# RhushabhVaghela/Custom-NVComp-with-ZSTD

Hardware: AMD Instinct MI355X
Metric: compress GB/s + ratio, 1 GB @ level 3, 64 KB chunks; libzstd round-trip OK (higher is better)
Workload: dtype u8; 1 GPU; C3: 16384 x 64 KiB chunks (1.00 GiB), level 3, independent frames; chunk_bytes=65536, chunks_total=16384, chunks_rank0=16384, level=3, parallelism=dp1 (contiguous chunk shards, RCCL all-gather of sizes inside the step), gathered_frame_bytes=388747049

## Files before the change

### custom-nvcomp-with-zstd_amd/csrc/zh_common.h

```cpp
#pragma once
#include <hip/hip_runtime.h>
#include <stdint.h>
#include "zstd_hip_params.h"
#include "zh_dict_ent.h"
#include "zh_block_plan.h"

typedef int16_t s16;
typedef int32_t s32;

#define ZH_STATS_LIT 0u
#define ZH_STATS_LL 256u
#define ZH_STATS_OF 320u
#define ZH_STATS_ML 384u
#define ZH_STATS_WORDS 448u

#define ZH_SEQ_CAP 13120u
#define ZH_SEQ_BYTES (ZH_SEQ_CAP * 8u)
#define ZH_K3_W 1u
#define ZH_K3_SEGS (21u * ZH_K3_W)
#define ZH_K3_SLOTS (64u * ZH_K3_W)
#define ZH_K3_RUN 16u
#define ZH_K3_SLOT(t, g) (3u * (g) + (t))
#define ZH_K3_TSTRIDE ZH_K3_RUN
#define ZH_K3_SEGLEN(nbseq) ((((nbseq) + ZH_K3_SEGS - 1u) / ZH_K3_SEGS + ZH_K3_RUN - 1u) & ~(ZH_K3_RUN - 1u))
// ... 29 lines not shown
  u8 *base;
  u32 *ctr;
  const u16 *dtab;
  u32 dtab_P;
  const u32 *dd_prev;
  const u32 *dd_head;
  u32 dd_pre, dd_split;
  u8 *deep_slots;
  u32 deep_nslots;
  const ZhDictEnt *dent;
  u32 *stats;
  __device__ u64 *seq(u32 b) const { return (u64 *)(base + (size_t)b * ZH_WS_BLOCK_BYTES); }
  __device__ u8 *lits(u32 b) const { return base + (size_t)b * ZH_WS_BLOCK_BYTES + ZH_SEQ_BYTES; }
  __device__ u32 *meta(u32 b) const { return (u32 *)(base + (size_t)b * ZH_WS_BLOCK_BYTES + ZH_SEQ_BYTES + ZH_LIT_BYTES); }
  __device__ u32 *dbg(u32 b) const { return meta(b) + 4; }
  __device__ u8 *fse(u32 b) const { return base + (size_t)b * ZH_WS_BLOCK_BYTES + ZH_SEQ_BYTES + ZH_LIT_BYTES + ZH_META_BYTES; }
  __device__ u32 *fsef(u32 b) const { return (u32 *)(fse(b) + ZH_FSE_FIELDS); }
};

#define ZH_DTAB_MARGIN 256u

struct ZhClassRanges {
  u32 range[ZH_NCLASSES][2];
  u32 ctr[4];
};
#define ZH_RANGE_CTR_DEEP 3u

__host__ __device__ __forceinline__ u32 zh_k3_magic(u32 L) { return ((1u << 24) + L - 1u) / L; }
__device__ __forceinline__ u32 zh_k3_index(u32 e, u32 t, u32 L, u32 m) {
  u32 const g = __umulhi(e << 8, m), r = e - g * L;
// ... 26 lines not shown
```

### custom-nvcomp-with-zstd_amd/csrc/zh_entropy.hip

```cpp
#include "zh_common.h"

namespace {

constexpr u32 K2_THREADS = 128;
constexpr u32 SW_WORDS = 184;

constexpr u32 OFF_SW = 0;
constexpr u32 OFF_HVAL = OFF_SW + 4 * SW_WORDS;
constexpr u32 OFF_HNB = OFF_HVAL + 2 * 256;
constexpr u32 OFF_MISC = OFF_HNB + 256;
constexpr u32 OFF_HIST = OFF_MISC + 4 * 64;
constexpr u32 OFF_HBUF = OFF_HIST + 4 * 256;
constexpr u32 OFF_SCR = OFF_HBUF + 768;
constexpr u32 OFF_U = OFF_SCR + 1024;
static_assert(OFF_U % 16 == 0, "alignment");
constexpr u32 OFF_NODES = OFF_U;
constexpr u32 U_HUF_END = OFF_NODES + 8 * 516;
constexpr u32 OFF_ST_LL = OFF_U;
constexpr u32 OFF_ST_OF = OFF_ST_LL + 1024;
constexpr u32 OFF_ST_ML = OFF_ST_OF + 512;
constexpr u32 OFF_SYM = OFF_ST_ML + 1024;
constexpr u32 SYM_OF = 36, SYM_ML = 68;
constexpr u32 OFF_TSYM = OFF_SYM + 976;
constexpr u32 OFF_NORM = OFF_TSYM + 512;
// ... 848 lines not shown
    sz[k] = (wave_sum(bits) + 1 + 7) >> 3;
    cs += sz[k];
  }
  u32 const fl = 1 + (nl > 31) + (nl > 4095);
  u32 const other = (cLit == 0 || cLit >= nl - minGain) ? fl + nl : cLit == 1 ? fl + 1 : lhSize + cLit;
  if (lhSize + cs > other) return false;
  wave_sync();
  ((u32 *)hnb)[lane] = ((const u32 *)dent->hnb)[lane];
  ((u32 *)hval)[lane] = ((const u32 *)dent->hval)[lane];
  ((u32 *)hval)[64 + lane] = ((const u32 *)dent->hval)[64 + lane];
  if (lane == 0) { ssz[0] = sz[0]; ssz[1] = sz[1]; ssz[2] = sz[2]; ssz[3] = sz[3]; ssz[4] = cs; }
  wave_sync();
  return true;
}

extern "C" __global__ __launch_bounds__(K2_THREADS) void zh_entropy_kernel(const ZhBlockDesc *__restrict__ blocks, ZhWorkspace ws, u32 window_log,
                                                                             u32 cfg_block_size, u64 *__restrict__ item_size,
                                                                             u32 *__restrict__ item_status, u32 *__restrict__ blk_size,
                                                                             const u8 *__restrict__ blk_level) {
  extern __shared__ __attribute__((aligned(16))) u8 smem_all[];
  u32 const wave = threadIdx.x >> 6;
  u8 *const smem = smem_all + wave * K2_W1;
  u32 *const xch = (u32 *)(smem_all + OFF_MISC) + 56;
  u32 *sw = (u32 *)(smem + OFF_SW);
  u32 *misc = (u32 *)(smem + OFF_MISC);
  u32 *hist = (u32 *)(smem + OFF_HIST);
  u16 *hval = (u16 *)(smem + OFF_HVAL);
  u8 *hnb = smem + OFF_HNB;
  u8 *hbuf = smem + OFF_HBUF;
  HufNode *nodes = (HufNode *)(smem + OFF_NODES);
  u16 *stLL = (u16 *)(smem + OFF_ST_LL), *stOF = (u16 *)(smem + OFF_ST_OF), *stML = (u16 *)(smem + OFF_ST_ML);
  FseSym *symLL = (FseSym *)(smem + OFF_SYM), *symOF = symLL + SYM_OF, *symML = symLL + SYM_ML;
  u8 *tsym = smem + OFF_TSYM;
  s16 *norm = (s16 *)(smem + OFF_NORM);
  u8 *wts = smem + OFF_WTS;
  SerialScratch *scr = (SerialScratch *)(smem + OFF_SCR);

  u32 const b = blockIdx.x, lane = lane_id();
  ZhBlockDesc const d = blocks[b];
  u32 const n = d.n;
  if (n == 0) return;
  const u32 *meta = ws.meta(b);
  u32 const nseq_raw = meta[0], nlit = meta[1], rle = meta[2] == 1u, k1hist = meta[2] == ZH_META_K1HIST;
  Out const o{d.dst, d.dst_cap};
  constexpr u32 DENT_FLAGS = ZH_F_FIRST | ZH_F_DICT | ZH_F_DICTENT;
  const ZhDictEnt *const dent = (d.flags & DENT_FLAGS) == DENT_FLAGS ? ws.dent : nullptr;
  u32 *const stats = (d.flags & ZH_F_STATS) ? ws.stats : nullptr;
  u32 const lit_min = stats ? 1u : (dent && !k1hist) ? ZH_DENT_LITERALS_MIN : ZH_COMPRESS_LITERALS_SIZE_MIN + 1u;
  if (wave == 0 && lane == 0) sw[0] = 0;
#ifdef ZH_STAMPS
  u64 stamp_prev = __builtin_amdgcn_s_memtime();
  u32 st[12] = {0, 0, 0, 0, 0, 0, 0, 0, 0, 0, 0, 0};
#endif
// ... 514 lines not shown
        total = finish_block(d, o, blk, op, false);
      }
    }
  }
  ZH_STAMP(8);
#ifdef ZH_STAMPS
  if (lane == 0) {
    u32 *dbg = ws.dbg(b);
    if (wave == 0) { for (int k = 0; k < 4; k++) dbg[6 + k] = st[k]; dbg[42] = st[11]; }
    else { for (int k = 4; k < 9; k++) dbg[6 + k] = st[k]; dbg[17] = st[9]; dbg[18] = st[10]; dbg[19] = nseq_raw; }
  }
#endif
  if (wave == 1 && !handoff) write_status(d, b, total, item_size, item_status, blk_size);
}

constexpr u32 K3_SEGS = ZH_K3_SEGS;
constexpr u32 K3_W = ZH_K3_W;
constexpr u32 K3_OCC = 8;
constexpr u32 K3_WARM = 128;
constexpr u32 K3_WAVES = K3_W == 1 ? 4 : K3_W;
constexpr u32 K3_BPW = K3_WAVES / K3_W;
constexpr u32 K3_TAB_STRIDE = (ZH_FSE_TAB_BYTES + 15) & ~15u;
constexpr u32 K3_LDS = K3_BPW * K3_TAB_STRIDE + 64;
constexpr u32 K3_BATCH = 16;
constexpr u32 K3_TABW = ZH_FSE_TAB_BYTES / 4;

__device__ __forceinline__ void k3_chain(ZhWorkspace ws, u32 bb, u8 *smem, u32 lane, u32 *xw) {
#ifdef ZH_STAMPS
  u64 const k3pre = __builtin_amdgcn_s_memtime();
  u64 const k3rt0 = __builtin_amdgcn_s_memrealtime();
// ... 118 lines not shown
    k3rerun += __builtin_popcountll(__ballot(active));
#endif
    if (active) {
      entry = ne;
      u32 s = ne;
      if (!pass(s, true)) x = s;
    }
  }
  if (g == K3_SEGS - 1 && lane < 3 * K3_SEGS) ff[ZH_FF_SLL + t] = x;
#ifdef ZH_STAMPS
  if (lane == 0) { u32 *dbg = ws.dbg(bb); dbg[46] = (u32)(__builtin_amdgcn_s_memtime() - k3t0); dbg[47] = k3rounds; dbg[48] = k3rerun; dbg[49] = nbSeq;
                   dbg[50] = (u32)(k3t0 - k3pre); dbg[51] = (u32)k3rt0; dbg[52] = (u32)__builtin_amdgcn_s_memrealtime(); }
#endif
}

extern "C" __global__ __launch_bounds__(64 * K3_WAVES) __attribute__((amdgpu_waves_per_eu(K3_OCC, 8))) void zh_fse_chain_kernel(const ZhBlockDesc *__restrict__ blocks, u32 nblocks, ZhWorkspace ws) {
  extern __shared__ __attribute__((aligned(16))) u8 smem_all[];
  u32 const bw = threadIdx.x / (64 * K3_W), lane = threadIdx.x % (64 * K3_W);
  u32 const bb = blockIdx.x * K3_BPW + bw;
  if (bb >= nblocks || blocks[bb].n == 0) return;
  if (ws.fsef(bb)[ZH_FF_NEED] == 0) return;
  k3_chain(ws, bb, smem_all + bw * K3_TAB_STRIDE, lane, (u32 *)(smem_all + K3_BPW * K3_TAB_STRIDE));
}

constexpr u32 KP_SW = 0, KP_DNB = 4 * SW_WORDS, KP_LDS = (KP_DNB + 4 * 128 + 15) & ~15u;
constexpr u32 K4_WAVES = 4;
constexpr u32 K4_PF = 1;

__device__ __forceinline__ void k4_pack(const ZhBlockDesc &d, ZhWorkspace ws, u32 b, u8 *smem, u32 lane, u64 *__restrict__ item_size,
                                        u32 *__restrict__ item_status, u32 *__restrict__ blk_size) {
  const u32 *ff = ws.fsef(b);
  u32 *sw = (u32 *)(smem + KP_SW);
  u32 *dNb = (u32 *)(smem + KP_DNB);
  const u8 *fz = ws.fse(b);
  if (lane < 36) dNb[lane] = ((const FseSym *)(fz + ZH_FT_SYLL))[lane].dNb;
  if (lane < 32) dNb[40 + lane] = ((const FseSym *)(fz + ZH_FT_SYOF))[lane].dNb;
  if (lane < 53) dNb[72 + lane] = ((const FseSym *)(fz + ZH_FT_SYML))[lane].dNb;
// ... 40 lines not shown
    }
    u32 v6[6] = {vOF, vML, vLL, ll, mlb, ob};
    u32 n6[6] = {nOF, nML, nLL, valid ? llbits : 0u, valid ? mlbits : 0u, ofc};
    sink_append<6>(bs, o, sw, v6, n6);
  }
  {
    u32 v3[3] = {sML, sOF, sLL};
    u32 n3[3] = {lane == 0 ? logML : 0u, lane == 0 ? logOF : 0u, lane == 0 ? logLL : 0u};
    sink_append<3>(bs, o, sw, v3, n3);
  }
  sink_close(bs, o, sw);
  u32 const total = finish_block(d, o, blk, bs.pos, false);
  write_status(d, b, total, item_size, item_status, blk_size);
}

extern "C" __global__ __launch_bounds__(64 * K4_WAVES) void zh_seq_pack_kernel(const ZhBlockDesc *__restrict__ blocks, u32 nblocks, ZhWorkspace ws,
                                                                               u64 *__restrict__ item_size, u32 *__restrict__ item_status,
                                                                               u32 *__restrict__ blk_size) {
  extern __shared__ __attribute__((aligned(16))) u8 smem_all[];
  u32 const wv = threadIdx.x >> 6, b = blockIdx.x * K4_WAVES + wv;
  if (b >= nblocks) return;
  ZhBlockDesc const d = blocks[b];
  if (d.n == 0 || ws.fsef(b)[ZH_FF_NEED] == 0) return;
  k4_pack(d, ws, b, smem_all + wv * KP_LDS, lane_id(), item_size, item_status, blk_size);
}

extern "C" u32 zh_entropy_lds_bytes() { return K2_LDS; }
#ifdef ZH_STAMPS
extern "C" __global__ void zh_read_hst(u32 *out) { for (int k = 0; k < 6; k++) { out[k] = g_hst[k]; g_hst[k] = 0; } }
extern "C" void zh_hst_host(u32 *out6) {
  u32 *d = nullptr;
  if (hipMalloc(&d, 24) != hipSuccess) return;
  hipLaunchKernelGGL(zh_read_hst, dim3(1), dim3(1), 0, 0, d);
  (void)hipMemcpy(out6, d, 24, hipMemcpyDeviceToHost);
  (void)hipFree(d);
}
#endif

namespace zh {
hipError_t entropy_init() {
  hipError_t e = hipFuncSetAttribute((const void *)zh_entropy_kernel, hipFuncAttributeMaxDynamicSharedMemorySize, (int)K2_LDS);
  if (e == hipSuccess) e = hipFuncSetAttribute((const void *)zh_fse_chain_kernel, hipFuncAttributeMaxDynamicSharedMemorySize, (int)K3_LDS);
  return e;
}
void entropy_launch(const ZhBlockDesc *d_descs, u32 nblocks, ZhWorkspace ws, u32 window_log, u32 cfg_block_size, u64 *d_item_size,
                    u32 *d_item_status, u32 *d_blk_size, const u8 *d_blk_level, hipStream_t stream) {
  hipLaunchKernelGGL(zh_entropy_kernel, dim3(nblocks), dim3(K2_THREADS), K2_LDS, stream, d_descs, ws, window_log, cfg_block_size, d_item_size,
                     d_item_status, d_blk_size, d_blk_level);
  u32 const g3 = (nblocks + K3_BPW - 1) / K3_BPW, g4 = (nblocks + K4_WAVES - 1) / K4_WAVES;
  hipLaunchKernelGGL(zh_fse_chain_kernel, dim3(g3), dim3(64 * K3_WAVES), K3_LDS, stream, d_descs, nblocks, ws);
  hipLaunchKernelGGL(zh_seq_pack_kernel, dim3(g4), dim3(64 * K4_WAVES), K4_WAVES * KP_LDS, stream, d_descs, nblocks, ws, d_item_size,
                     d_item_status, d_blk_size);
}
}
```

### custom-nvcomp-with-zstd_amd/csrc/zh_host.cpp

```cpp
#include <hip/hip_runtime.h>
#include <dlfcn.h>
#if defined(__SANITIZE_ADDRESS__)
#define ZH_DLOPEN_DEEPBIND 0
#elif defined(__has_feature)
#if __has_feature(address_sanitizer)
#define ZH_DLOPEN_DEEPBIND 0
#endif
#endif
#ifndef ZH_DLOPEN_DEEPBIND
#define ZH_DLOPEN_DEEPBIND RTLD_DEEPBIND
#endif

#include <algorithm>
#include <chrono>
#include <cstring>
#include <mutex>
#include <new>
#include <vector>

#include "cuda_zstd_adaptive.h"
#include "cuda_zstd_hybrid.h"
#include "cuda_zstd_manager.h"
#include "cuda_zstd_nvcomp.h"
#include "zh_adaptive.h"
// ... 284 lines not shown
struct WsLayout {
  size_t descs, items, blk_size, item_size, item_status, staging, counter, blocks, deep, deep_slots, total;
  size_t ldm_table, ldm_skey, ldm_sslot, ldm_scount, ldm_rec;
  size_t rank, blk_level, ranges;
  BatchShape shape;
  explicit WsLayout(const BatchShape &s) : shape(s) {
    size_t const nblocks = s.nblocks, nitems = s.nitems, cells = s.ldm_cells;
    size_t o = 0;
    auto take = [&o](size_t bytes) { size_t const at = o; o = align256(o + bytes); return at; };
    descs = take(nblocks * sizeof(ZhBlockDesc));
    items = take(nitems * sizeof(ZhItemDesc));
    blk_size = take(nblocks * 4);
    item_size = take(nitems * 8);
    item_status = take(nitems * 4);
    staging = take(s.staged ? nblocks * (size_t)ZH_STAGE_SLOT : 0);
    counter = take(4);
    blocks = take(nblocks * (size_t)ZH_WS_BLOCK_BYTES);
    deep_slots = s.deep ? std::min(nblocks, (size_t)ZH_DEEP_SLOTS_MAX) : 0;
    deep = take(deep_slots * ZH_DEEP_SLOT_BYTES);
    ldm_table = take(cells ? sizeof(u64) << s.ldm_tlog : 0);
    ldm_skey = take(cells * ZH_LDM_CELL_SAMPLES * sizeof(u64));
    ldm_sslot = take(cells * ZH_LDM_CELL_SAMPLES * sizeof(u32));
    ldm_scount = take(cells * sizeof(u32));
    ldm_rec = take(cells * sizeof(ZhLdmRecord));
    rank = take(s.levels ? nitems * 4 : 0);
    blk_level = take(s.levels ? nblocks : 0);
    ranges = take(s.levels ? sizeof(ZhClassRanges) : 0);
    total = o + 256;
  }
};

// ... 168 lines not shown
    a.dict = d;
    a.dict_n = n;
    a.dict_off = (u32)off;
    a.dict_id = id;
  }
};

ZhBatch bind_batch(const WsLayout &L, u8 *base, const DevDict *dd, const CompressionConfig &c, u32 *stats = nullptr) {
  if (dd && !dd->n) dd = nullptr;
  ZhBatch b{};
  b.descs = (ZhBlockDesc *)(base + L.descs);
  b.items = (ZhItemDesc *)(base + L.items);
  b.item_size = (u64 *)(base + L.item_size);
  b.item_status = (u32 *)(base + L.item_status);
  b.blk_size = (u32 *)(base + L.blk_size);
  b.nblocks = (u32)L.shape.nblocks;
  b.nitems = (u32)L.shape.nitems;
  b.block_size = c.block_size;
  b.level = c.level;
  b.gather = L.shape.staged;
  b.checksum = c.checksum != ChecksumPolicy::NO_COMPUTE_NO_VERIFY;
  b.window_log = L.shape.levels ? 0u : c.window_log;
  const ZhDictEnt *const dent = dd ? dd->dent(c) : nullptr;
  b.plan.flags = (b.checksum ? ZH_F_CHECKSUM : 0u) | (dent ? ZH_F_DICTENT : 0u) | (stats ? ZH_F_STATS : 0u);
  b.plan.hist = L.shape.levels || c.window_log >= ZH_HIST_WINDOW_LOG;
  if (dd) {
    b.plan.dict = dd->content();
    b.plan.dict_n = (u32)dd->content_n();
    b.plan.dict_id = dd->id;
  }
// ... 1998 lines not shown
}
long long cuda_zstd_hip_ldm_plan(cuda_zstd_manager_t *m, const void *d_src, size_t size, unsigned int *host_records, size_t capacity,
                                 void *workspace, size_t workspace_size, hipStream_t stream) {
  if (!m || !m->manager) return -1;
  size_t n = 0;
  Status const s = m->manager->ldm_plan(d_src, size, host_records, capacity, &n, workspace, workspace_size, stream);
  if (s != Status::SUCCESS) { (void)c_err(s); return -1; }
  return (long long)n;
}
void cuda_zstd_hip_ldm_profile(int on, double *ms) {
  double const t = zh::ldm_profile(on != 0);
  if (ms) *ms = t;
}
void cuda_zstd_hip_profile_enable(int on) { zh::profile_enable(on != 0); }
int cuda_zstd_hip_profile_collect(double *ms3) { return zh::profile_collect(ms3); }

struct cuda_zstd_stream_t {
  std::unique_ptr<ZstdStreamingManager> m;
};
cuda_zstd_stream_t *cuda_zstd_stream_create(int level) {
  if (!is_valid_compression_level(level)) return nullptr;
  try {
    auto *h = new cuda_zstd_stream_t;
    h->m.reset(new ZstdStreamingManager(CompressionConfig::from_level(level)));
    return h;
  } catch (...) {
    return nullptr;
  }
}
void cuda_zstd_stream_destroy(cuda_zstd_stream_t *s) { delete s; }
// ... 179 lines not shown
```

### custom-nvcomp-with-zstd_amd/csrc/zh_launch.h

```cpp
#pragma once
#include "zh_common.h"
#include "zh_ldm.h"

struct ZhDecArgs {
  const void *const *in_ptrs;
  const void *one_in;
  u64 one_in_size;
  void *one_out;
  const size_t *in_sizes;
  void *const *out_ptrs;
  const size_t *out_caps;
  u64 out_cap_all;
  size_t *out_sizes;
  u32 *statuses;
  u8 *ws;
  u64 slot_bytes;
  u32 lit_bytes, block_cap, seq_cap, nvcomp_codes;
  u32 ho_off;
  const u8 *dict;
  u64 dict_n;
  u32 dict_off;
  u32 dict_id;
};
#define ZH_DEC_HANDOFF_BYTES 5376u

struct ZhBatch {
  ZhBlockDesc *descs;
  ZhItemDesc *items;
  u64 *item_size;
  u32 *item_status;
  u32 *blk_size;
  ZhBatchPlan plan;
  ZhWorkspace ws;
  u32 *rank;
  u8 *blk_level;
  ZhClassRanges *ranges;
  u32 nblocks, nitems;
  u32 window_log, block_size;
  int level;
  bool gather, checksum;
};

struct ZhPlanArrays {
  const void *const *in_ptrs;
  const size_t *in_sizes;
  void *const *out_ptrs;
  const int *levels;
};

namespace zh {
u32 dec_lds_bytes();
hipError_t launch_decompress(const ZhDecArgs &a, u32 nitems, hipStream_t stream);
hipError_t launch_decompress_sizes(const ZhDecArgs &a, u32 nitems, hipStream_t stream);
hipError_t init_kernels();
u32 lz_lds_bytes();
u32 entropy_lds_bytes();
hipError_t lz_dict_tables(const u8 *content, size_t cn, u16 *out, u32 *tmp32, u32 &P, hipStream_t stream);
hipError_t lz_deep_dict_tables(const u8 *content, size_t cn, u8 *stg, u32 *dprev, u32 *dhead, u32 &P, u32 &split, hipStream_t stream);
hipError_t launch_compress(const ZhBatch &b, hipStream_t stream);
void profile_enable(bool on);
int profile_collect(double *totals);
#define ZH_RANK_MAX_ITEMS (1u << 20)
hipError_t launch_plan(const ZhBatch &b, const ZhPlanArrays &a, hipStream_t stream);
hipError_t ldm_launch(const u8 *src, u64 size, u32 ncells, u32 table_log, u32 max_dist, u32 flags, u64 *table, u64 *skey, u32 *sslot,
                      u32 *scount, ZhBlockDesc *descs, u8 *staging, u32 *blk_size, ZhLdmRecord *rec, hipStream_t stream);
double ldm_profile(bool on);
}
```

### custom-nvcomp-with-zstd_amd/csrc/zh_plan.hip

```cpp
#include "zh_common.h"
#include "zh_launch.h"
#include "zh_scan.h"
#include "zh_xxh64.h"

#include <mutex>
#include <vector>

extern "C" u32 zh_lz_lds_bytes();
extern "C" u32 zh_entropy_lds_bytes();
namespace zh {
hipError_t lz_init();
void lz_launch(const ZhBlockDesc *d_descs, u32 nblocks, ZhWorkspace ws, u32 mode, hipStream_t stream);
void lz_launch_ranged(const ZhBlockDesc *d_descs, u32 nblocks, ZhWorkspace ws, ZhClassRanges *d_ranges, hipStream_t stream);
hipError_t lz_deep_init();
hipError_t lz_deep_launch(const ZhBlockDesc *d_descs, u32 nblocks, ZhWorkspace ws, int level, hipStream_t stream);
hipError_t lz_deep_launch_ranged(const ZhBlockDesc *d_descs, u32 nblocks, ZhWorkspace ws, ZhClassRanges *d_ranges, const u8 *d_blk_level,
                                 hipStream_t stream);
hipError_t entropy_init();
void entropy_launch(const ZhBlockDesc *d_descs, u32 nblocks, ZhWorkspace ws, u32 window_log, u32 cfg_block_size, u64 *d_item_size,
                    u32 *d_item_status, u32 *d_blk_size, const u8 *d_blk_level, hipStream_t stream);
}

__device__ inline void zh_plan_block(const ZhBatch &B, const ZhPlanArrays &a, u32 i, u32 k, u32 b, int level, bool valid) {
  ZhPlanItem const it{(const u8 *)a.in_ptrs[i], a.in_sizes[i], i, level, (u8 *)a.out_ptrs[i]};
  ZhBlockDesc d = zh_block_desc(B.plan, it, k, b);
  if (!valid) d.n = 0;
  B.descs[b] = d;
  if (k != 0) return;
  bool invalid;
  B.items[i] = zh_item_desc(B.plan, it, b, &invalid);
  if (invalid || !valid) { B.item_size[i] = 0; B.item_status[i] = ZH_ST_INVALID; }
}

extern "C" __global__ void zh_plan_kernel(ZhBatch B, ZhPlanArrays a) {
  u32 const t = blockIdx.x * blockDim.x + threadIdx.x, bpi = B.nblocks / B.nitems;
// ... 46 lines not shown
    cr->range[tid][1] = b1 * bpi;
    if (tid <= ZH_CLASS_DEEP0) cr->ctr[tid] = b0 * bpi;
  }
}

extern "C" __global__ void zh_plan_levels_kernel(ZhBatch B, ZhPlanArrays a) {
  u32 const t = blockIdx.x * blockDim.x + threadIdx.x, bpi = B.nblocks / B.nitems;
  if (t >= B.nblocks) return;
  u32 const i = t / bpi, k = t % bpi, b = B.rank[i] * bpi + k;
  int const level = a.levels[i];
  bool const valid = ZH_LEVEL_VALID(level);
  zh_plan_block(B, a, i, k, b, level, valid);
  B.blk_level[b] = valid ? (u8)level : (u8)0;
}
static_assert(ZH_LEVEL_WINDOW_LOG(1) >= ZH_HIST_WINDOW_LOG, "every level's frames may reach the previous block");

extern "C" __global__ __launch_bounds__(256) void zh_gather_kernel(const ZhItemDesc *__restrict__ items, const ZhBlockDesc *__restrict__ descs,
                                                                    const u32 *__restrict__ blk_size, u64 *item_size, u32 *item_status) {
  u32 const b = blockIdx.x, tid = threadIdx.x;
  ZhBlockDesc const d = descs[b];
  if (d.n == 0 && !(d.flags & ZH_F_LDM)) return;
  ZhItemDesc const id = items[d.item];
  if (id.nblocks <= 1) return;
  u32 const k = b - id.first_block;
  __shared__ u64 part[2][4];
  __shared__ u32 badp[4];
  u64 pre = 0, tot = 0;
  u32 bad = 0;
  for (u32 j = tid; j < id.nblocks; j += 256) {
    u32 const s = blk_size[id.first_block + j];
// ... 37 lines not shown
  if (size + 4 > id.cap) {
    if (lane == 0) item_status[it] = ZH_ST_TOO_SMALL;
    return;
  }
  if (lane < 4) id.dst[size + lane] = (u8)(h >> (8 * lane));
  if (lane == 0) item_size[it] = size + 4;
}

namespace zh {

hipError_t init_kernels() {
  hipError_t e = lz_init();
  if (e != hipSuccess) return e;
  e = lz_deep_init();
  if (e != hipSuccess) return e;
  return entropy_init();
}

u32 lz_lds_bytes() { return zh_lz_lds_bytes(); }
u32 entropy_lds_bytes() { return zh_entropy_lds_bytes(); }

namespace {
struct ProfState {
  std::mutex mu;
  bool on = false;
  std::vector<hipEvent_t> pool;
  std::vector<std::vector<hipEvent_t>> pending;
};
ProfState &prof() {
  static ProfState p;
// ... 20 lines not shown
  int n = 0;
  for (auto &ev : p.pending) {
    (void)hipEventSynchronize(ev[3]);
    float a = 0, b = 0, c = 0;
    (void)hipEventElapsedTime(&a, ev[0], ev[1]);
    (void)hipEventElapsedTime(&b, ev[1], ev[2]);
    (void)hipEventElapsedTime(&c, ev[2], ev[3]);
    totals[0] += a; totals[1] += b; totals[2] += c;
    for (auto e : ev) p.pool.push_back(e);
    n++;
  }
  p.pending.clear();
  return n;
}

hipError_t launch_compress(const ZhBatch &b, hipStream_t stream) {
  if (b.nblocks == 0) return hipSuccess;
  std::vector<hipEvent_t> ev;
  {
    std::lock_guard<std::mutex> g(prof().mu);
    if (prof().on) for (int k = 0; k < 4; k++) ev.push_back(prof_event());
  }
  if (!ev.empty()) (void)hipEventRecord(ev[0], stream);
  if (b.ranges) {
    lz_launch_ranged(b.descs, b.nblocks, b.ws, b.ranges, stream);
    hipError_t const e = lz_deep_launch_ranged(b.descs, b.nblocks, b.ws, b.ranges, b.blk_level, stream);
    if (e != hipSuccess) return e;
  } else if (b.level >= ZH_DEEP_LEVEL) {
    (void)hipMemsetAsync(b.ws.ctr, 0, 4, stream);
    hipError_t const e = lz_deep_launch(b.descs, b.nblocks, b.ws, b.level, stream);
    if (e != hipSuccess) return e;
  } else {
    (void)hipMemsetAsync(b.ws.ctr, 0, 4, stream);
    lz_launch(b.descs, b.nblocks, b.ws, (u32)ZH_K1_MODE(b.level), stream);
  }
  if (!ev.empty()) (void)hipEventRecord(ev[1], stream);
  entropy_launch(b.descs, b.nblocks, b.ws, b.window_log, b.block_size, b.item_size, b.item_status, b.blk_size, b.blk_level, stream);
  if (!ev.empty()) (void)hipEventRecord(ev[2], stream);
  if (b.gather && b.nitems)
    hipLaunchKernelGGL(zh_gather_kernel, dim3(b.nblocks), dim3(256), 0, stream, b.items, b.descs, b.blk_size, b.item_size, b.item_status);
  if (b.checksum && b.nitems)
    hipLaunchKernelGGL(zh_checksum_kernel, dim3(b.nitems), dim3(64), 0, stream, b.items, b.descs, b.item_size, b.item_status);
  if (!ev.empty()) {
    (void)hipEventRecord(ev[3], stream);
    std::lock_guard<std::mutex> g(prof().mu);
    prof().pending.push_back(ev);
  }
  return hipGetLastError();
}

hipError_t launch_plan(const ZhBatch &b, const ZhPlanArrays &a, hipStream_t stream) {
  if (!b.nblocks) return hipSuccess;
// ... 13 lines not shown
```

### custom-nvcomp-with-zstd_amd/cuda_zstd/__init__.py

```python
from __future__ import annotations

import ctypes
import os
from typing import List, Sequence

_HERE = os.path.dirname(os.path.abspath(__file__))
LIB_PATH = os.environ.get("CUDA_ZSTD_HIP_LIB") or os.path.join(os.path.dirname(_HERE), "libcuda_zstd_hip.so")

OK, INVALID, OOM, DEVICE_ERROR, CORRUPT, TOO_SMALL, CHECKSUM, COMPRESSION = 0, 2, 3, 4, 6, 7, 10, 12

_lib = None


class ZstdError(RuntimeError):
    def __init__(self, code: int, what: str = ""):
        self.code = code
        super().__init__(f"{what}: {error_string(code)} (code {code})")


def lib() -> ctypes.CDLL:
    global _lib
    if _lib is None:
        if not os.path.exists(LIB_PATH):
            raise ImportError(f"{LIB_PATH} not found: build it with __graft_entry__.build() (make -C custom-nvcomp-with-zstd_amd)")
# ... 1005 lines not shown
    rc = lib().cuda_zstd_extract_metadata(ptr, n, ctypes.byref(lv), ctypes.byref(us), ctypes.byref(did), ctypes.byref(ck))
    del keep
    if rc:
        raise ZstdError(rc, "cuda_zstd_extract_metadata")
    return {"level": lv.value, "uncompressed_size": us.value, "dictionary_id": did.value, "checksum": bool(ck.value)}


def profile_enable(on: bool = True) -> None:
    lib().cuda_zstd_hip_profile_enable(1 if on else 0)


def profile_collect():
    ms = (ctypes.c_double * 3)()
    n = lib().cuda_zstd_hip_profile_collect(ms)
    return n, list(ms)
```

### include/cuda_zstd_capi.h

```cpp
#ifndef CUDA_ZSTD_CAPI_H_
#define CUDA_ZSTD_CAPI_H_

#include <hip/hip_runtime_api.h>
#include <stddef.h>

#ifdef __cplusplus
extern "C" {
#endif

typedef struct cuda_zstd_manager_t cuda_zstd_manager_t;
typedef struct cuda_zstd_dict_t cuda_zstd_dict_t;

cuda_zstd_manager_t *cuda_zstd_create_manager(int compression_level);
void cuda_zstd_destroy_manager(cuda_zstd_manager_t *manager);
int cuda_zstd_compress(cuda_zstd_manager_t *manager, const void *src, size_t src_size, void *dst, size_t *dst_size,
                       void *workspace, size_t workspace_size, hipStream_t stream);
int cuda_zstd_decompress(cuda_zstd_manager_t *manager, const void *src, size_t src_size, void *dst, size_t *dst_size,
                         void *workspace, size_t workspace_size, hipStream_t stream);
size_t cuda_zstd_get_compress_workspace_size(cuda_zstd_manager_t *manager, size_t src_size);
size_t cuda_zstd_get_decompress_workspace_size(cuda_zstd_manager_t *manager, size_t compressed_size);
cuda_zstd_dict_t *cuda_zstd_train_dictionary(const void **samples, const size_t *sample_sizes, size_t num_samples, size_t dict_size);
cuda_zstd_dict_t *cuda_zstd_train_dictionary_params(const void **samples, const size_t *sample_sizes, size_t num_samples,
                                                    size_t dict_size, unsigned k, unsigned d);
size_t cuda_zstd_train_dictionary_device_get_temp_size(size_t total_sample_bytes, size_t num_samples, size_t dict_size, unsigned k);
// ... 149 lines not shown
int cuda_zstd_adaptive_select_level(const void *d_data, size_t size, size_t sample_bytes, int preference,
                                    cuda_zstd_adaptive_stats_t *h_out, hipStream_t stream);
int cuda_zstd_adaptive_finalize_host(const unsigned *hist256, unsigned sample_size, unsigned repeated_pairs, unsigned max_run_length,
                                     unsigned pattern_score, int preference, cuda_zstd_adaptive_stats_t *out);

int cuda_zstd_set_long_distance(cuda_zstd_manager_t *manager, int enable, unsigned window_log, unsigned hash_log);
int cuda_zstd_set_dict_entropy(cuda_zstd_manager_t *manager, int enable);
int cuda_zstd_set_checksum(cuda_zstd_manager_t *manager, int enable);
long long cuda_zstd_hip_ldm_plan(cuda_zstd_manager_t *manager, const void *d_src, size_t size, unsigned int *host_records, size_t capacity,
                                 void *workspace, size_t workspace_size, hipStream_t stream);
void cuda_zstd_hip_ldm_profile(int on, double *ms);

const char *cuda_zstd_hip_version(void);
void cuda_zstd_hip_profile_enable(int on);
int cuda_zstd_hip_profile_collect(double *ms3);
void cuda_zstd_hip_dict_train_profile(int on, double *ms3);
unsigned int cuda_zstd_hip_kernel_lds_bytes(int which);

#ifdef __cplusplus
}
#endif
#endif
```

Measured before the change: 91.55 GB/s.

## Schedule entropy kernels over blocks sorted by estimated cost

Adds a key, counting-sort and scatter pass after LZ matching that buckets blocks by a cost estimate from their metadata (sequence and literal counts). The three entropy kernels then dispatch workgroups through this order, so the heaviest blocks start first and the tail imbalance should shrink. The ordering only runs above a block-count threshold and when more than one bucket is occupied. It costs three extra small launches, including a single-workgroup sort, and one extra indirection per block, and it reuses the blk_size buffer as sort scratch.

```diff
diff --git a/custom-nvcomp-with-zstd_amd/csrc/zh_common.h b/custom-nvcomp-with-zstd_amd/csrc/zh_common.h
--- a/custom-nvcomp-with-zstd_amd/csrc/zh_common.h
+++ b/custom-nvcomp-with-zstd_amd/csrc/zh_common.h
@@ -67,6 +67,16 @@
   __device__ u8 *lits(u32 b) const { return base + (size_t)b * ZH_WS_BLOCK_BYTES + ZH_SEQ_BYTES; }
   __device__ u32 *meta(u32 b) const { return (u32 *)(base + (size_t)b * ZH_WS_BLOCK_BYTES + ZH_SEQ_BYTES + ZH_LIT_BYTES); }
   __device__ u32 *dbg(u32 b) const { return meta(b) + 4; }
+  __device__ u32 *order(u32 s) const { return meta(s) + 3; }
+  __device__ bool order_useful() const {
+    u64 const active = ((u64)ctr[2] << 32 | ctr[1]) & ~(1ull << 63);
+    return (active & (active - 1)) != 0;
+  }
+  template <bool ORD>
+  __device__ u32 dispatch(u32 s) const {
+    if constexpr (ORD) return order_useful() ? *order(s) : s;
+    else return s;
+  }
   __device__ u8 *fse(u32 b) const { return base + (size_t)b * ZH_WS_BLOCK_BYTES + ZH_SEQ_BYTES + ZH_LIT_BYTES + ZH_META_BYTES; }
   __device__ u32 *fsef(u32 b) const { return (u32 *)(fse(b) + ZH_FSE_FIELDS); }
 };
diff --git a/custom-nvcomp-with-zstd_amd/csrc/zh_entropy.hip b/custom-nvcomp-with-zstd_amd/csrc/zh_entropy.hip
--- a/custom-nvcomp-with-zstd_amd/csrc/zh_entropy.hip
+++ b/custom-nvcomp-with-zstd_amd/csrc/zh_entropy.hip
@@ -886,10 +886,10 @@
   return true;
 }
 
-extern "C" __global__ __launch_bounds__(K2_THREADS) void zh_entropy_kernel(const ZhBlockDesc *__restrict__ blocks, ZhWorkspace ws, u32 window_log,
-                                                                             u32 cfg_block_size, u64 *__restrict__ item_size,
-                                                                             u32 *__restrict__ item_status, u32 *__restrict__ blk_size,
-                                                                             const u8 *__restrict__ blk_level) {
+template <bool ORD>
+__device__ __forceinline__ void k2_block(const ZhBlockDesc *__restrict__ blocks, ZhWorkspace ws, u32 window_log, u32 cfg_block_size,
+                                         u64 *__restrict__ item_size, u32 *__restrict__ item_status, u32 *__restrict__ blk_size,
+                                         const u8 *__restrict__ blk_level) {
   extern __shared__ __attribute__((aligned(16))) u8 smem_all[];
   u32 const wave = threadIdx.x >> 6;
   u8 *const smem = smem_all + wave * K2_W1;
@@ -908,7 +908,7 @@
   u8 *wts = smem + OFF_WTS;
   SerialScratch *scr = (SerialScratch *)(smem + OFF_SCR);
 
-  u32 const b = blockIdx.x, lane = lane_id();
+  u32 const b = ws.dispatch<ORD>(blockIdx.x), lane = lane_id();
   ZhBlockDesc const d = blocks[b];
   u32 const n = d.n;
   if (n == 0) return;
@@ -1453,6 +1453,19 @@
   if (wave == 1 && !handoff) write_status(d, b, total, item_size, item_status, blk_size);
 }
 
+extern "C" __global__ __launch_bounds__(K2_THREADS) void zh_entropy_kernel(const ZhBlockDesc *__restrict__ blocks, ZhWorkspace ws, u32 window_log,
+                                                                             u32 cfg_block_size, u64 *__restrict__ item_size,
+                                                                             u32 *__restrict__ item_status, u32 *__restrict__ blk_size,
+                                                                             const u8 *__restrict__ blk_level) {
+  k2_block<false>(blocks, ws, window_log, cfg_block_size, item_size, item_status, blk_size, blk_level);
+}
+extern "C" __global__ __launch_bounds__(K2_THREADS) void zh_entropy_ordered_kernel(const ZhBlockDesc *__restrict__ blocks, ZhWorkspace ws,
+                                                                                     u32 window_log, u32 cfg_block_size, u64 *__restrict__ item_size,
+                                                                                     u32 *__restrict__ item_status, u32 *__restrict__ blk_size,
+                                                                                     const u8 *__restrict__ blk_level) {
+  k2_block<true>(blocks, ws, window_log, cfg_block_size, item_size, item_status, blk_size, blk_level);
+}
+
 constexpr u32 K3_SEGS = ZH_K3_SEGS;
 constexpr u32 K3_W = ZH_K3_W;
 constexpr u32 K3_OCC = 8;
@@ -1601,13 +1614,22 @@
 #endif
 }
 
-extern "C" __global__ __launch_bounds__(64 * K3_WAVES) __attribute__((amdgpu_waves_per_eu(K3_OCC, 8))) void zh_fse_chain_kernel(const ZhBlockDesc *__restrict__ blocks, u32 nblocks, ZhWorkspace ws) {
+template <bool ORD>
+__device__ __forceinline__ void k3_workgroup(const ZhBlockDesc *__restrict__ blocks, u32 nblocks, ZhWorkspace ws) {
   extern __shared__ __attribute__((aligned(16))) u8 smem_all[];
   u32 const bw = threadIdx.x / (64 * K3_W), lane = threadIdx.x % (64 * K3_W);
-  u32 const bb = blockIdx.x * K3_BPW + bw;
-  if (bb >= nblocks || blocks[bb].n == 0) return;
+  u32 const slot = blockIdx.x * K3_BPW + bw;
+  if (slot >= nblocks) return;
+  u32 const bb = ws.dispatch<ORD>(slot);
+  if (blocks[bb].n == 0) return;
   if (ws.fsef(bb)[ZH_FF_NEED] == 0) return;
   k3_chain(ws, bb, smem_all + bw * K3_TAB_STRIDE, lane, (u32 *)(smem_all + K3_BPW * K3_TAB_STRIDE));
+}
+extern "C" __global__ __launch_bounds__(64 * K3_WAVES) __attribute__((amdgpu_waves_per_eu(K3_OCC, 8))) void zh_fse_chain_kernel(const ZhBlockDesc *__restrict__ blocks, u32 nblocks, ZhWorkspace ws) {
+  k3_workgroup<false>(blocks, nblocks, ws);
+}
+extern "C" __global__ __launch_bounds__(64 * K3_WAVES) __attribute__((amdgpu_waves_per_eu(K3_OCC, 8))) void zh_fse_chain_ordered_kernel(const ZhBlockDesc *__restrict__ blocks, u32 nblocks, ZhWorkspace ws) {
+  k3_workgroup<true>(blocks, nblocks, ws);
 }
 
 constexpr u32 KP_SW = 0, KP_DNB = 4 * SW_WORDS, KP_LDS = (KP_DNB + 4 * 128 + 15) & ~15u;
@@ -1678,15 +1700,26 @@
   write_status(d, b, total, item_size, item_status, blk_size);
 }
 
+template <bool ORD>
+__device__ __forceinline__ void k4_workgroup(const ZhBlockDesc *__restrict__ blocks, u32 nblocks, ZhWorkspace ws, u64 *__restrict__ item_size,
+                                             u32 *__restrict__ item_status, u32 *__restrict__ blk_size) {
+  extern __shared__ __attribute__((aligned(16))) u8 smem_all[];
+  u32 const wv = threadIdx.x >> 6, slot = blockIdx.x * K4_WAVES + wv;
+  if (slot >= nblocks) return;
+  u32 const b = ws.dispatch<ORD>(slot);
+  ZhBlockDesc const d = blocks[b];
+  if (d.n == 0 || ws.fsef(b)[ZH_FF_NEED] == 0) return;
+  k4_pack(d, ws, b, smem_all + wv * KP_LDS, lane_id(), item_size, item_status, blk_size);
+}
 extern "C" __global__ __launch_bounds__(64 * K4_WAVES) void zh_seq_pack_kernel(const ZhBlockDesc *__restrict__ blocks, u32 nblocks, ZhWorkspace ws,
                                                                                u64 *__restrict__ item_size, u32 *__restrict__ item_status,
                                                                                u32 *__restrict__ blk_size) {
-  extern __shared__ __attribute__((aligned(16))) u8 smem_all[];
-  u32 const wv = threadIdx.x >> 6, b = blockIdx.x * K4_WAVES + wv;
-  if (b >= nblocks) return;
-  ZhBlockDesc const d = blocks[b];
-  if (d.n == 0 || ws.fsef(b)[ZH_FF_NEED] == 0) return;
-  k4_pack(d, ws, b, smem_all + wv * KP_LDS, lane_id(), item_size, item_status, blk_size);
+  k4_workgroup<false>(blocks, nblocks, ws, item_size, item_status, blk_size);
+}
+extern "C" __global__ __launch_bounds__(64 * K4_WAVES) void zh_seq_pack_ordered_kernel(const ZhBlockDesc *__restrict__ blocks, u32 nblocks,
+                                                                                       ZhWorkspace ws, u64 *__restrict__ item_size,
+                                                                                       u32 *__restrict__ item_status, u32 *__restrict__ blk_size) {
+  k4_workgroup<true>(blocks, nblocks, ws, item_size, item_status, blk_size);
 }
 
 extern "C" u32 zh_entropy_lds_bytes() { return K2_LDS; }
@@ -1704,16 +1737,19 @@
 namespace zh {
 hipError_t entropy_init() {
   hipError_t e = hipFuncSetAttribute((const void *)zh_entropy_kernel, hipFuncAttributeMaxDynamicSharedMemorySize, (int)K2_LDS);
+  if (e == hipSuccess) e = hipFuncSetAttribute((const void *)zh_entropy_ordered_kernel, hipFuncAttributeMaxDynamicSharedMemorySize, (int)K2_LDS);
   if (e == hipSuccess) e = hipFuncSetAttribute((const void *)zh_fse_chain_kernel, hipFuncAttributeMaxDynamicSharedMemorySize, (int)K3_LDS);
+  if (e == hipSuccess) e = hipFuncSetAttribute((const void *)zh_fse_chain_ordered_kernel, hipFuncAttributeMaxDynamicSharedMemorySize, (int)K3_LDS);
   return e;
 }
 void entropy_launch(const ZhBlockDesc *d_descs, u32 nblocks, ZhWorkspace ws, u32 window_log, u32 cfg_block_size, u64 *d_item_size,
-                    u32 *d_item_status, u32 *d_blk_size, const u8 *d_blk_level, hipStream_t stream) {
-  hipLaunchKernelGGL(zh_entropy_kernel, dim3(nblocks), dim3(K2_THREADS), K2_LDS, stream, d_descs, ws, window_log, cfg_block_size, d_item_size,
-                     d_item_status, d_blk_size, d_blk_level);
+                    u32 *d_item_status, u32 *d_blk_size, const u8 *d_blk_level, bool ordered, hipStream_t stream) {
+  hipLaunchKernelGGL(ordered ? zh_entropy_ordered_kernel : zh_entropy_kernel, dim3(nblocks), dim3(K2_THREADS), K2_LDS, stream, d_descs, ws,
+                     window_log, cfg_block_size, d_item_size, d_item_status, d_blk_size, d_blk_level);
   u32 const g3 = (nblocks + K3_BPW - 1) / K3_BPW, g4 = (nblocks + K4_WAVES - 1) / K4_WAVES;
-  hipLaunchKernelGGL(zh_fse_chain_kernel, dim3(g3), dim3(64 * K3_WAVES), K3_LDS, stream, d_descs, nblocks, ws);
-  hipLaunchKernelGGL(zh_seq_pack_kernel, dim3(g4), dim3(64 * K4_WAVES), K4_WAVES * KP_LDS, stream, d_descs, nblocks, ws, d_item_size,
-                     d_item_status, d_blk_size);
-}
-}
+  hipLaunchKernelGGL(ordered ? zh_fse_chain_ordered_kernel : zh_fse_chain_kernel, dim3(g3), dim3(64 * K3_WAVES), K3_LDS, stream, d_descs, nblocks,
+                     ws);
+  hipLaunchKernelGGL(ordered ? zh_seq_pack_ordered_kernel : zh_seq_pack_kernel, dim3(g4), dim3(64 * K4_WAVES), K4_WAVES * KP_LDS, stream, d_descs,
+                     nblocks, ws, d_item_size, d_item_status, d_blk_size);
+}
+}
diff --git a/custom-nvcomp-with-zstd_amd/csrc/zh_host.cpp b/custom-nvcomp-with-zstd_amd/csrc/zh_host.cpp
--- a/custom-nvcomp-with-zstd_amd/csrc/zh_host.cpp
+++ b/custom-nvcomp-with-zstd_amd/csrc/zh_host.cpp
@@ -322,7 +322,7 @@
     item_size = take(nitems * 8);
     item_status = take(nitems * 4);
     staging = take(s.staged ? nblocks * (size_t)ZH_STAGE_SLOT : 0);
-    counter = take(4);
+    counter = take(12);
     blocks = take(nblocks * (size_t)ZH_WS_BLOCK_BYTES);
     deep_slots = s.deep ? std::min(nblocks, (size_t)ZH_DEEP_SLOTS_MAX) : 0;
     deep = take(deep_slots * ZH_DEEP_SLOT_BYTES);
@@ -521,6 +521,7 @@
   b.item_size = (u64 *)(base + L.item_size);
   b.item_status = (u32 *)(base + L.item_status);
   b.blk_size = (u32 *)(base + L.blk_size);
+  b.order_scratch = L.shape.ldm_cells ? nullptr : b.blk_size;
   b.nblocks = (u32)L.shape.nblocks;
   b.nitems = (u32)L.shape.nitems;
   b.block_size = c.block_size;
@@ -2549,6 +2550,8 @@
 }
 void cuda_zstd_hip_profile_enable(int on) { zh::profile_enable(on != 0); }
 int cuda_zstd_hip_profile_collect(double *ms3) { return zh::profile_collect(ms3); }
+void cuda_zstd_hip_order_threshold(long long min_blocks) { zh::order_threshold(min_blocks); }
+int cuda_zstd_hip_order_debug_read(unsigned *out5, unsigned cap_slots) { return out5 ? zh::order_debug_read(out5, cap_slots) : -1; }
 
 struct cuda_zstd_stream_t {
   std::unique_ptr<ZstdStreamingManager> m;
diff --git a/custom-nvcomp-with-zstd_amd/csrc/zh_launch.h b/custom-nvcomp-with-zstd_amd/csrc/zh_launch.h
--- a/custom-nvcomp-with-zstd_amd/csrc/zh_launch.h
+++ b/custom-nvcomp-with-zstd_amd/csrc/zh_launch.h
@@ -30,6 +30,7 @@
   u64 *item_size;
   u32 *item_status;
   u32 *blk_size;
+  u32 *order_scratch;
   ZhBatchPlan plan;
   ZhWorkspace ws;
   u32 *rank;
@@ -60,6 +61,8 @@
 hipError_t launch_compress(const ZhBatch &b, hipStream_t stream);
 void profile_enable(bool on);
 int profile_collect(double *totals);
+void order_threshold(long long min_blocks);
+int order_debug_read(u32 *out, u32 cap_slots);
 #define ZH_RANK_MAX_ITEMS (1u << 20)
 hipError_t launch_plan(const ZhBatch &b, const ZhPlanArrays &a, hipStream_t stream);
 hipError_t ldm_launch(const u8 *src, u64 size, u32 ncells, u32 table_log, u32 max_dist, u32 flags, u64 *table, u64 *skey, u32 *sslot,
diff --git a/custom-nvcomp-with-zstd_amd/csrc/zh_plan.hip b/custom-nvcomp-with-zstd_amd/csrc/zh_plan.hip
--- a/custom-nvcomp-with-zstd_amd/csrc/zh_plan.hip
+++ b/custom-nvcomp-with-zstd_amd/csrc/zh_plan.hip
@@ -3,6 +3,8 @@
 #include "zh_scan.h"
 #include "zh_xxh64.h"
 
+#include <algorithm>
+#include <cstddef>
 #include <mutex>
 #include <vector>
 
@@ -18,7 +20,7 @@
                                  hipStream_t stream);
 hipError_t entropy_init();
 void entropy_launch(const ZhBlockDesc *d_descs, u32 nblocks, ZhWorkspace ws, u32 window_log, u32 cfg_block_size, u64 *d_item_size,
-                    u32 *d_item_status, u32 *d_blk_size, const u8 *d_blk_level, hipStream_t stream);
+                    u32 *d_item_status, u32 *d_blk_size, const u8 *d_blk_level, bool ordered, hipStream_t stream);
 }
 
 __device__ inline void zh_plan_block(const ZhBatch &B, const ZhPlanArrays &a, u32 i, u32 k, u32 b, int level, bool valid) {
@@ -95,6 +97,80 @@
   B.blk_level[b] = valid ? (u8)level : (u8)0;
 }
 static_assert(ZH_LEVEL_WINDOW_LOG(1) >= ZH_HIST_WINDOW_LOG, "every level's frames may reach the previous block");
+
+#define ZH_ORDER_THREADS 1024u
+#define ZH_ORDER_BUCKETS 64u
+#define ZH_ORDER_SHIFT 8u
+#define ZH_ORDER_MAX_BLOCKS (1u << 19)
+#define ZH_ORDER_CELLS (ZH_ORDER_THREADS * ZH_ORDER_BUCKETS)
+#define ZH_ORDER_CNT_BYTES (2u * (ZH_ORDER_CELLS + 2u * (ZH_ORDER_CELLS >> 6)))
+#define ZH_ORDER_LDS (ZH_ORDER_CNT_BYTES + 4u * ZH_ORDER_THREADS + 4u * (ZH_ORDER_THREADS / 64u))
+static_assert(ZH_ORDER_BUCKETS == 64u, "a thread scans one 64-cell run");
+static_assert(64u * (ZH_ORDER_MAX_BLOCKS / ZH_ORDER_THREADS) <= 65535u, "a run's prefix fits a u16 cell");
+static_assert(ZH_ORDER_CNT_BYTES % 4u == 0 && ZH_ORDER_LDS <= 160u * 1024u, "the matrix fits the CU's LDS");
+
+extern "C" __global__ __launch_bounds__(256) void zh_order_key_kernel(const ZhBlockDesc *__restrict__ blocks, u32 nblocks, ZhWorkspace ws,
+                                                                       u32 *__restrict__ key) {
+  u32 const i = blockIdx.x * 256u + threadIdx.x;
+  u32 bucket = ZH_ORDER_BUCKETS - 1u;
+  if (i < nblocks && blocks[i].n != 0) {
+    const u32 *meta = ws.meta(i);
+    u32 const q = min((meta[0] + (meta[1] >> 4)) >> ZH_ORDER_SHIFT, ZH_ORDER_BUCKETS - 2u);
+    if (meta[2] != 1u) bucket = ZH_ORDER_BUCKETS - 2u - q;
+  }
+  if (i < nblocks) key[i] = bucket;
+  __shared__ u32 seen[2];
+  if (threadIdx.x < 2) seen[threadIdx.x] = 0;
+  __syncthreads();
+  atomicOr(&seen[bucket >> 5], 1u << (bucket & 31u));
+  __syncthreads();
+  if (threadIdx.x < 2 && seen[threadIdx.x]) atomicOr(&ws.ctr[1 + threadIdx.x], seen[threadIdx.x]);
+}
+
+__device__ __forceinline__ u32 zh_order_cell(u32 bucket, u32 tid) {
+  u32 const f = bucket * ZH_ORDER_THREADS + tid;
+  return f + 2u * (f >> 6);
+}
+
+extern "C" __global__ __launch_bounds__(ZH_ORDER_THREADS) void zh_order_kernel(u32 *__restrict__ key, u32 nblocks, ZhWorkspace ws) {
+  extern __shared__ __attribute__((aligned(16))) u8 order_lds[];
+  if (!ws.order_useful()) return;
+  u16 *const cnt = (u16 *)order_lds;
+  u32 *const tbase = (u32 *)(order_lds + ZH_ORDER_CNT_BYTES), *const wsum = tbase + ZH_ORDER_THREADS;
+  u32 const tid = threadIdx.x;
+  u32 const per = (nblocks + ZH_ORDER_THREADS - 1) / ZH_ORDER_THREADS;
+  u32 const i0 = min(tid * per, nblocks), i1 = min(i0 + per, nblocks);
+  for (u32 w = tid; w < ZH_ORDER_CNT_BYTES / 4u; w += ZH_ORDER_THREADS) ((u32 *)cnt)[w] = 0;
+  __syncthreads();
+  for (u32 i = i0; i < i1; i++) cnt[zh_order_cell(min(key[i], ZH_ORDER_BUCKETS - 1u), tid)]++;
+  __syncthreads();
+  u16 *const run = cnt + 66u * tid;
+  u32 sum = 0;
+  for (u32 j = 0; j < 64; j++) {
+    u32 const c = run[j];
+    run[j] = (u16)sum;
+    sum += c;
+  }
+  u32 const inc = wave_scan_incl(sum);
+  if ((tid & 63u) == 63u) wsum[tid >> 6] = inc;
+  __syncthreads();
+  u32 before = 0;
+  for (u32 w = 0; w < (tid >> 6); w++) before += wsum[w];
+  tbase[tid] = before + inc - sum;
+  __syncthreads();
+  for (u32 i = i0; i < i1; i++) {
+    u32 const bucket = min(key[i], ZH_ORDER_BUCKETS - 1u), c = zh_order_cell(bucket, tid);
+    key[i] = tbase[(bucket * ZH_ORDER_THREADS + tid) >> 6] + cnt[c];
+    cnt[c]++;
+  }
+}
+
+extern "C" __global__ __launch_bounds__(256) void zh_order_scatter_kernel(const u32 *__restrict__ rank, u32 nblocks, ZhWorkspace ws) {
+  u32 const i = blockIdx.x * 256u + threadIdx.x;
+  if (i >= nblocks || !ws.order_useful()) return;
+  u32 const r = rank[i];
+  if (r < nblocks) *ws.order(r) = i;
+}
 
 extern "C" __global__ __launch_bounds__(256) void zh_gather_kernel(const ZhItemDesc *__restrict__ items, const ZhBlockDesc *__restrict__ descs,
                                                                     const u32 *__restrict__ blk_size, u64 *item_size, u32 *item_status) {
@@ -162,6 +238,8 @@
   if (e != hipSuccess) return e;
   e = lz_deep_init();
   if (e != hipSuccess) return e;
+  e = hipFuncSetAttribute((const void *)zh_order_kernel, hipFuncAttributeMaxDynamicSharedMemorySize, (int)ZH_ORDER_LDS);
+  if (e != hipSuccess) return e;
   return entropy_init();
 }
 
@@ -212,8 +290,62 @@
   return n;
 }
 
+namespace {
+constexpr u32 kOrderMinBlocks = 8192;
+struct OrderState {
+  std::mutex mu;
+  u32 min_blocks = kOrderMinBlocks;
+  bool armed = false;
+  const ZhBlockDesc *descs = nullptr;
+  const u8 *base = nullptr;
+  const u32 *ctr = nullptr;
+  u32 nblocks = 0;
+};
+OrderState &order_state() {
+  static OrderState s;
+  return s;
+}
+}
+
+void order_threshold(long long min_blocks) {
+  OrderState &s = order_state();
+  std::lock_guard<std::mutex> g(s.mu);
+  s.min_blocks = min_blocks < 0 ? kOrderMinBlocks : (u32)std::min<long long>(min_blocks, 0xFFFFFFFFll);
+  s.armed = min_blocks >= 0;
+  s.descs = nullptr; s.base = nullptr; s.ctr = nullptr; s.nblocks = 0;
+}
+
+int order_debug_read(u32 *out, u32 cap_slots) {
+  OrderState &s = order_state();
+  std::lock_guard<std::mutex> g(s.mu);
+  if (!s.nblocks) return 0;
+  if (hipDeviceSynchronize() != hipSuccess) return -1;
+  u32 mask[2] = {0, 0};
+  if (hipMemcpy(mask, s.ctr + 1, 8, hipMemcpyDeviceToHost) != hipSuccess) return -1;
+  u64 const active = ((u64)mask[1] << 32 | mask[0]) & ~(1ull << 63);
+  if (!(active & (active - 1))) return 0;
+  u32 const n = std::min(cap_slots, s.nblocks);
+  std::vector<u32> sizes(n), meta((size_t)n * 4);
+  const u8 *const meta0 = s.base + ZH_SEQ_BYTES + ZH_LIT_BYTES;
+  if (n && (hipMemcpy2D(sizes.data(), 4, (const u8 *)s.descs + offsetof(ZhBlockDesc, n), sizeof(ZhBlockDesc), 4, n, hipMemcpyDeviceToHost) != hipSuccess ||
+            hipMemcpy2D(meta.data(), 16, meta0, ZH_WS_BLOCK_BYTES, 16, n, hipMemcpyDeviceToHost) != hipSuccess))
+    return -1;
+  for (u32 i = 0; i < n; i++) {
+    out[5 * i] = sizes[i];
+    for (u32 k = 0; k < 4; k++) out[5 * i + 1 + k] = meta[4 * (size_t)i + k];
+  }
+  return (int)s.nblocks;
+}
+
 hipError_t launch_compress(const ZhBatch &b, hipStream_t stream) {
   if (b.nblocks == 0) return hipSuccess;
+  bool ordered;
+  {
+    OrderState &s = order_state();
+    std::lock_guard<std::mutex> g(s.mu);
+    ordered = b.order_scratch && b.nblocks > s.min_blocks && b.nblocks <= ZH_ORDER_MAX_BLOCKS;
+    if (ordered && s.armed) { s.descs = b.descs; s.base = b.ws.base; s.ctr = b.ws.ctr; s.nblocks = b.nblocks; }
+  }
   std::vector<hipEvent_t> ev;
   {
     std::lock_guard<std::mutex> g(prof().mu);
@@ -221,19 +353,26 @@
   }
   if (!ev.empty()) (void)hipEventRecord(ev[0], stream);
   if (b.ranges) {
+    if (ordered) (void)hipMemsetAsync(b.ws.ctr + 1, 0, 8, stream);
     lz_launch_ranged(b.descs, b.nblocks, b.ws, b.ranges, stream);
     hipError_t const e = lz_deep_launch_ranged(b.descs, b.nblocks, b.ws, b.ranges, b.blk_level, stream);
     if (e != hipSuccess) return e;
   } else if (b.level >= ZH_DEEP_LEVEL) {
-    (void)hipMemsetAsync(b.ws.ctr, 0, 4, stream);
+    (void)hipMemsetAsync(b.ws.ctr, 0, ordered ? 12 : 4, stream);
     hipError_t const e = lz_deep_launch(b.descs, b.nblocks, b.ws, b.level, stream);
     if (e != hipSuccess) return e;
   } else {
-    (void)hipMemsetAsync(b.ws.ctr, 0, 4, stream);
+    (void)hipMemsetAsync(b.ws.ctr, 0, ordered ? 12 : 4, stream);
     lz_launch(b.descs, b.nblocks, b.ws, (u32)ZH_K1_MODE(b.level), stream);
   }
   if (!ev.empty()) (void)hipEventRecord(ev[1], stream);
-  entropy_launch(b.descs, b.nblocks, b.ws, b.window_log, b.block_size, b.item_size, b.item_status, b.blk_size, b.blk_level, stream);
+  if (ordered) {
+    dim3 const per_slot((b.nblocks + 255) / 256);
+    hipLaunchKernelGGL(zh_order_key_kernel, per_slot, dim3(256), 0, stream, b.descs, b.nblocks, b.ws, b.order_scratch);
+    hipLaunchKernelGGL(zh_order_kernel, dim3(1), dim3(ZH_ORDER_THREADS), ZH_ORDER_LDS, stream, b.order_scratch, b.nblocks, b.ws);
+    hipLaunchKernelGGL(zh_order_scatter_kernel, per_slot, dim3(256), 0, stream, b.order_scratch, b.nblocks, b.ws);
+  }
+  entropy_launch(b.descs, b.nblocks, b.ws, b.window_log, b.block_size, b.item_size, b.item_status, b.blk_size, b.blk_level, ordered, stream);
   if (!ev.empty()) (void)hipEventRecord(ev[2], stream);
   if (b.gather && b.nitems)
     hipLaunchKernelGGL(zh_gather_kernel, dim3(b.nblocks), dim3(256), 0, stream, b.items, b.descs, b.blk_size, b.item_size, b.item_status);
diff --git a/custom-nvcomp-with-zstd_amd/cuda_zstd/__init__.py b/custom-nvcomp-with-zstd_amd/cuda_zstd/__init__.py
--- a/custom-nvcomp-with-zstd_amd/cuda_zstd/__init__.py
+++ b/custom-nvcomp-with-zstd_amd/cuda_zstd/__init__.py
@@ -1043,3 +1043,20 @@
     ms = (ctypes.c_double * 3)()
     n = lib().cuda_zstd_hip_profile_collect(ms)
     return n, list(ms)
+
+
+def set_order_threshold(min_blocks=None) -> None:
+    f = lib().cuda_zstd_hip_order_threshold
+    f.restype, f.argtypes = None, [ctypes.c_longlong]
+    f(-1 if min_blocks is None else int(min_blocks))
+
+
+def order_debug_read(cap_slots: int = 1 << 20):
+    f = lib().cuda_zstd_hip_order_debug_read
+    f.restype, f.argtypes = ctypes.c_int, [ctypes.POINTER(ctypes.c_uint), ctypes.c_uint]
+    buf = (ctypes.c_uint * (5 * cap_slots))()
+    n = f(buf, cap_slots)
+    if n < 0:
+        raise RuntimeError("cuda_zstd_hip_order_debug_read failed")
+    n = min(n, cap_slots)
+    return [tuple(buf[5 * k:5 * k + 5]) for k in range(n)]
diff --git a/include/cuda_zstd_capi.h b/include/cuda_zstd_capi.h
--- a/include/cuda_zstd_capi.h
+++ b/include/cuda_zstd_capi.h
@@ -187,6 +187,8 @@
 const char *cuda_zstd_hip_version(void);
 void cuda_zstd_hip_profile_enable(int on);
 int cuda_zstd_hip_profile_collect(double *ms3);
+void cuda_zstd_hip_order_threshold(long long min_blocks);
+int cuda_zstd_hip_order_debug_read(unsigned *out5, unsigned cap_slots);
 void cuda_zstd_hip_dict_train_profile(int on, double *ms3);
 unsigned int cuda_zstd_hip_kernel_lds_bytes(int which);
 
```

After: 93.34 GB/s, median of 6. 1.02x the previous value.
